# bobocode/lmono

Measured on AMD Instinct MI355X. Metric: KITTI HDL-64 scans/sec (scanRegistration + laserOdometry), higher is better.
Workload: dtype f32 features / f64 solve

## Files before the change

### lmono_amd/csrc/corr_flat.hip

```cpp
#include "batch.hpp"

namespace lmono {

#ifndef LMONO_CF_T
#define LMONO_CF_T 128
#endif
constexpr int kCfT = LMONO_CF_T;
constexpr int kCfBlocks = kMaxQueries / kCfT;
static_assert(kMaxQueries % kCfT == 0, "feature capacity must be a multiple of the workgroup size");
static_assert(kCfBlocks == kThinBlocks, "k_lm_solve skips the records of the workgroups a thinned lead-in pair does not run");
#ifndef LMONO_CF_PER
#define LMONO_CF_PER 6
#endif
#ifndef LMONO_CF_WAVES
#define LMONO_CF_WAVES 1
#endif
constexpr int kCfPer = LMONO_CF_PER;
constexpr int kCfPool = kCfT * kCfPer;
#ifndef LMONO_R0_PLANE
#define LMONO_R0_PLANE 0.25f
#define LMONO_R0_EDGE 0.7f
#endif
constexpr float kCfR0Edge = LMONO_R0_EDGE, kCfR0Plane = LMONO_R0_PLANE;
constexpr int kCfC = 4;
// ... 329 lines not shown
            elev_window(rr, elo, ehi);
            cf_window_extend(el, elo, ehi, v1, v2);
            const int pieces = cf_arc_pieces(a);
            const int nreq = max(v2 - v1 + 1, 0) * pieces;
            int slot = nreq > 0 ? atomicAdd(&L.n_pool[par], nreq) : 0;
            if (slot + nreq <= kCfPool) {
                posted = true;
                const int n0 = min(a.nb, kAzBins - a.a0);
                const unsigned int w0 = cf_request_line(0, a.a0, n0, tid), w1 = cf_request_line(0, 0, a.nb - n0, tid);
                for (int v = v1; v <= v2; v++) {
                    const float4 ev = el[v];
                    const bool meet = !(ev.y < elo || ev.x > ehi);
                    L.req[slot++] = meet ? (w0 | (unsigned int)v) : 0u;
                    if (pieces == 2) L.req[slot++] = meet ? (w1 | (unsigned int)v) : 0u;
                }
            } else {
                for (int t = slot; t < kCfPool; t++) L.req[t] = 0u;
            }
        }
        __syncthreads();
        CF_STAMP(cf_acc[0])
        const int n_chunks = cf_sweep<false>(L, par, n_edge_owner, tg, pts_c, pts_s, cf_t, cf_acc);
        par ^= 1;
        __syncthreads();
        CF_STAMP(cf_acc[2])
#ifdef LMONO_TILE_PROF
        if (tid == 0) { cf_acc[6] += 1; cf_acc[8] += (unsigned long long)n_chunks; }
#else
        (void)n_chunks;
#endif
        if (alive && posted) {
            const unsigned long long best = L.best[tid];
            if (best != ~0ull) {
                const float bd = __uint_as_float((unsigned int)(best >> 32));
                if (bd <= (rr * 0.9999f) * (rr * 0.9999f) || rr >= 5.0f) alive = false;
                else r = sqrtf(bd) * 1.0005f + 1e-3f;
            } else {
                if (rr >= 5.0f) alive = false;
                else r = rr * 2.5f;
            }
        }
        CF_STAMP(cf_acc[3])
        if (!__syncthreads_or(alive ? 1 : 0)) break;
    }
    if (alive) { alive = false; deferred = true; }

    const unsigned long long nn = L.best[tid];
    const unsigned long long thr = pack_fu(25.0f, 0u);
    bool walking = qi < nq && n_last > 0 && !deferred && nn != ~0ull && (double)__uint_as_float((unsigned int)(nn >> 32)) < 25.0;
    const int closest = (int)((unsigned int)(nn & 0xffffffffull) >> 7);
    const int ra = (int)(nn & 127ull);
    if (walking) {
        L.closest[tid] = (closest << 7) | ra;
        L.wlo[tid] = ra - 3 >= 0 ? L.lle[cl][ra - 3] + 1 : 0;
        L.whi[tid] = ra + 3 <= 65 ? L.fge[cl][ra + 3] : n_last;
    }
    const float rad[4] = { walk_radius(0, rho), walk_radius(1, rho), walk_radius(2, rho), walk_radius(3, rho) };
    int wpass = 0;
    unsigned long long same = thr, other = thr;
    float r_seed = -1.0f;
    if (walking && prev.w != 0 && prev.x == closest) {
        const int i_o = edge ? prev.y : prev.z;
        const float4 po = cloud[i_o];
        float d = dist2f(po.x, po.y, po.z, qx, qy, qz);
        if (!edge) { const float4 ps = cloud[prev.y]; d = fmaxf(d, dist2f(ps.x, ps.y, ps.z, qx, qy, qz)); }
        if (d < 24.0f) r_seed = sqrtf(d) * 1.002f + 1e-3f;
    }
    for (int round = 0; round < kCfWalkRounds; round++) {
#ifdef LMONO_TILE_PROF
        my_rounds += walking ? 1 : 0;
#endif
        bool posted = false;
        if (walking) {
            while (wpass > 0 && wpass < 4 && rad[wpass] <= rad[wpass - 1]) wpass++;
            if (wpass >= 4) walking = false;
        }
        const bool seeded = r_seed > 0.0f;
        const float r_now = seeded ? r_seed : rad[wpass < 4 ? wpass : 3];
        if (walking) {
            CfArc a;
            cf_arc(r_now, rho, th, a);
            const int wv1 = max(ra - 2, 0), wv2 = min(ra + 2, 65);
            const int nreq = (wv2 - wv1 + 1 - (edge ? 1 : 0)) * cf_arc_pieces(a);
            int slot = atomicAdd(&L.n_pool[par], nreq);
            if (slot + nreq <= kCfPool) {
                posted = true;
                L.same[tid] = thr; L.other[tid] = thr;
                for (int v = wv1; v <= wv2; v++) if (!(edge && v == ra)) cf_post_line(L.req, slot, a, v, tid);
            } else
                for (int t = slot; t < kCfPool; t++) L.req[t] = 0u;
        }
        __syncthreads();
        CF_STAMP(cf_acc[0])
        const int n_chunks = cf_sweep<true>(L, par, n_edge_owner, tg, pts_c, pts_s, cf_t, cf_acc);
        par ^= 1;
        __syncthreads();
        CF_STAMP(cf_acc[2])
#ifdef LMONO_TILE_PROF
        if (tid == 0) { cf_acc[7] += 1; cf_acc[9] += (unsigned long long)n_chunks; }
#else
        (void)n_chunks;
#endif
        if (walking && posted) {
            same = L.same[tid]; other = L.other[tid];
            if (!seeded && r_now >= 5.0f) walking = false;
            else {
                const unsigned long long lim = pack_fu(r_now * r_now * 0.998f, 0u);
                if (other < lim && (edge || same < lim)) walking = false;
                else if (seeded) r_seed = -1.0f;
                else {
                    wpass++;
                    while (wpass < 4 && rad[wpass] <= rad[wpass - 1]) wpass++;
                    if (other < thr && (edge || same < thr)) {
                        const float d = edge ? __uint_as_float((unsigned int)(other >> 32)) : fmaxf(__uint_as_float((unsigned int)(other >> 32)), __uint_as_float((unsigned int)(same >> 32)));
                        const float rt = sqrtf(d) * 1.002f + 1e-3f;
                        if (wpass < 4 && rt < rad[wpass] && d < 24.0f) r_seed = rt;
                    }
                }
            }
        }
        CF_STAMP(cf_acc[3])
        if (!__syncthreads_or(walking ? 1 : 0)) break;
    }
#ifdef LMONO_TILE_PROF
    {
        const int mr = __syncthreads_or(0) * 0 + my_rounds;
        __shared__ int s_maxr, s_sumr;
        if (tid == 0) { s_maxr = 0; s_sumr = 0; }
        __syncthreads();
        atomicMax(&s_maxr, mr); atomicAdd(&s_sumr, mr);
        __syncthreads();
        if (tid == 0) { cf_acc[17] = (unsigned long long)s_maxr; cf_acc[18] = (unsigned long long)s_sumr; }
    }
    if (tid == 0 && stats) { atomicAdd(&stats[1], 1ull); for (int i = 0; i < 20; i++) atomicAdd(&stats[2 + i], cf_acc[i]); }
#endif
    if (qi >= nq) return;
    if (deferred || walking) { cf_defer(wl, c, qi); return; }
    int4 rres = make_int4(-1, -1, -1, 0);
    int closest_out = -1;
    if (n_last > 0 && nn != ~0ull && (double)__uint_as_float((unsigned int)(nn >> 32)) < 25.0) {
        closest_out = closest;
        const int i_other = other < thr ? seq_to_index((unsigned int)(other & 0xffffffffull), closest) : -1;
        if (edge) { if (i_other >= 0) rres = make_int4(closest, i_other, -1, 1); }
        else {
            const int i_same = same < thr ? seq_to_index((unsigned int)(same & 0xffffffffull), closest) : -1;
            if (i_same >= 0 && i_other >= 0) rres = make_int4(closest, i_same, i_other, 2);
        }
    }
    ((int4 *)o.corr + (size_t)c * kMaxQueries)[qi] = rres;
    if (outer == 0 && seed_c) seed_c[qi] = closest_out;
    float4 A = make_float4(0.f, 0.f, 0.f, 0.f), B = A, C = A;
    if (rres.w != 0) { A = cloud[rres.x]; B = cloud[rres.y]; if (rres.z >= 0) C = cloud[rres.z]; }
    fp.w = __int_as_float(rres.w);
    float4 *rec = o.crec + ((size_t)c * kMaxQueries + qi) * 4;
    rec[0] = fp; rec[1] = A; rec[2] = B; rec[3] = C;
}

}
```

### lmono_amd/csrc/odometry.hip

```cpp
#include "batch.hpp"

namespace lmono {

constexpr float kCell = 1.0f;
constexpr float kInvCell = 1.0f;
constexpr int kMaxShell = 6;
constexpr int kCoordOff = 1 << 20;
constexpr int kRunMaxCount = 32767;
__device__ __forceinline__ int pack_run(int start, int count) { return start | (count << 17); }

__device__ __forceinline__ unsigned long long cell_key(int cx, int cy, int cz)
{
    return ((unsigned long long)(unsigned int)(cx + kCoordOff) << 42) |
           ((unsigned long long)(unsigned int)(cy + kCoordOff) << 21) |
           (unsigned long long)(unsigned int)(cz + kCoordOff);
}
__device__ __forceinline__ unsigned int hash_key(unsigned long long k)
{
    const unsigned int cz = (unsigned int)(k & 0x1fffffull), cy = (unsigned int)((k >> 21) & 0x1fffffull), cx = (unsigned int)(k >> 42);
    unsigned int h = (cx * 73856093u) ^ (cy * 19349663u) ^ (cz * 83492791u);
    h ^= h >> 15;
    return h;
}

struct GridRef {
    const GridCell *cell;
    const float4 *pts;
    int mask;
};

constexpr int kGridPage = 16384;
constexpr int kGridPar = 2;
constexpr int kGridLds = kGridPage * 8;
constexpr unsigned int kEmptyKey32 = 0xffffffffu;

__device__ __forceinline__ unsigned int grid_next(unsigned int sl, unsigned int pmask) { return (sl & ~pmask) | ((sl + 1) & pmask); }

__device__ __forceinline__ bool cell_key32(int cx, int cy, int cz, unsigned int &k)
{
    const unsigned int ux = (unsigned int)(cx + 1024), uy = (unsigned int)(cy + 1024), uz = (unsigned int)(cz + 512);
    k = ux | (uy << 11) | (uz << 22);
    return ux < 2048u && uy < 2048u && uz < 1023u;
}
__device__ __forceinline__ unsigned int hash_cell(int cx, int cy, int cz)
{
    unsigned int h = ((unsigned int)(cx + kCoordOff) * 73856093u) ^ ((unsigned int)(cy + kCoordOff) * 19349663u) ^ ((unsigned int)(cz + kCoordOff) * 83492791u);
    h ^= h >> 15;
    return h;
}
__device__ __forceinline__ unsigned long long key32_to_64(unsigned int k)
{
    return cell_key((int)(k & 2047u) - 1024, (int)((k >> 11) & 2047u) - 1024, (int)(k >> 22) - 512);
}

#ifdef LMONO_DIAG_SEARCH
__global__ __launch_bounds__(1024) void k_grid_build(BatchView b)
{
    const int s = b.scan0 + blockIdx.x;
    const bool surf = blockIdx.y > 0;
    const int tid = threadIdx.x, lane = tid & 63, wave = tid >> 6;
    const int n = b.feat_n[s * 4 + (surf ? 3 : 1)];
    const int Tcap = surf ? kSurfTable : kCornerTable;
    int T = next_pow2(n + 1);
    if (T < 1024) T = 1024;
    GridCell *cell = surf ? b.sg_cell + (size_t)s * kSurfTable : b.cg_cell + (size_t)s * kCornerTable;
    const int p0 = surf ? (int)blockIdx.y - 1 : 0, pstep = surf ? kGridPar : 1;
    if (T > Tcap) {
        if (p0 == 0) {
            for (int i = tid; i < 1024; i += 1024) { GridCell e; e.key = kEmptyKey; e.start = 0; e.cnt = 0; cell[i] = e; }
            if (tid == 0) { b.grid_mask[s * 2 + (surf ? 1 : 0)] = 1023; atomicOr(&b.status[s], kStatusGridOverflow); }
        }
        return;
    }
    const int P = T < kGridPage ? T : kGridPage, n_pages = T / P, pshift = __ffs(P) - 1;
    if (p0 >= n_pages) return;
    if (tid == 0 && p0 == 0) b.grid_mask[s * 2 + (surf ? 1 : 0)] = T - 1;
    const float4 *src = surf ? b.less_flat + b.off[s] : b.less_sharp + (size_t)s * kMaxLessSharp;
    float4 *dst = surf ? b.sg_pts + b.off[s] : b.cg_pts + (size_t)s * kMaxLessSharp;
    extern __shared__ __align__(16) unsigned int g_lds[];
    unsigned int *keys = g_lds;
    int *cnt = (int *)(g_lds + kGridPage);
    __shared__ int s_wsum[16], s_before, s_fail, s_occ;
    const unsigned int pm = (unsigned int)(P - 1);

    for (int p = p0; p < n_pages; p += pstep) {
        for (int i = tid; i < P; i += 1024) { keys[i] = kEmptyKey32; cnt[i] = 0; }
        if (tid == 0) { s_before = 0; s_fail = 0; s_occ = 0; }
        __syncthreads();
#pragma unroll
        for (int pass = 0; pass < 2; pass++) {
            int before = 0;
            bool fail = false;
            float4 nxt[4];
#pragma unroll
            for (int q = 0; q < 4; q++) { const int i = wave * 256 + 64 * q + lane; nxt[q] = i < n ? src[i] : make_float4(0.f, 0.f, 0.f, 0.f); }
            for (int t0 = wave * 256; t0 < n; t0 += 16 * 256) {
                unsigned int k32[4], sl[4];
                float4 pt[4];
                bool mine[4], head[4];
                int hl[4], len[4], base[4];
#pragma unroll
                for (int q = 0; q < 4; q++) {
                    pt[q] = nxt[q];
                    const int i = t0 + 16 * 256 + 64 * q + lane;
                    nxt[q] = i < n ? src[i] : make_float4(0.f, 0.f, 0.f, 0.f);
                }
#pragma unroll
                for (int q = 0; q < 4; q++) {
                    const int i = t0 + 64 * q + lane;
                    const int cx = (int)floorf(pt[q].x * kInvCell), cy = (int)floorf(pt[q].y * kInvCell), cz = (int)floorf(pt[q].z * kInvCell);
                    const bool ok = cell_key32(cx, cy, cz, k32[q]);
                    const unsigned int h = hash_cell(cx, cy, cz) & (unsigned int)(T - 1);
                    const int pg = (int)(h >> pshift);
                    sl[q] = h & pm;
                    mine[q] = i < n && pg == p;
                    if (i < n && pg < p) before++;
                    if (mine[q] && !ok) { fail = true; mine[q] = false; }
                }
#pragma unroll
                for (int q = 0; q < 4; q++) {
                    const unsigned int prev = (unsigned int)__shfl_up((int)k32[q], 1);
                    const unsigned long long mm = __ballot(mine[q]);
                    head[q] = mine[q] && (lane == 0 || !((mm >> (lane - 1)) & 1ull) || k32[q] != prev);
                    const unsigned long long hm = __ballot(head[q]);
                    hl[q] = 63 - __clzll((long long)(hm & ((2ull << lane) - 1ull)));
                    const unsigned long long stop = hm | ~mm;
                    const unsigned long long rest = lane < 63 ? stop >> (lane + 1) : 0ull;
                    len[q] = rest ? __ffsll((long long)rest) : 64 - lane;
                }
                unsigned int o4[4];
#pragma unroll
                for (int q = 0; q < 4; q++)
                    o4[q] = head[q] ? (pass == 0 ? atomicCAS(&keys[sl[q]], kEmptyKey32, k32[q]) : keys[sl[q]]) : k32[q];
#pragma unroll
                for (int q = 0; q < 4; q++) {
                    if (head[q]) {
                        unsigned int o = o4[q];
                        int tries = 0;
                        while (!(o == k32[q] || (pass == 0 && o == kEmptyKey32))) {
                            if (++tries >= P || (pass == 1 && o == kEmptyKey32)) { fail = true; head[q] = false; break; }
                            sl[q] = (sl[q] + 1) & pm;
                            o = pass == 0 ? atomicCAS(&keys[sl[q]], kEmptyKey32, k32[q]) : keys[sl[q]];
                        }
                    }
                }
#pragma unroll
                for (int q = 0; q < 4; q++) base[q] = head[q] ? atomicAdd(&cnt[sl[q]], len[q]) : -1;
                if (pass == 1) {
#pragma unroll
                    for (int q = 0; q < 4; q++) {
                        const int i = t0 + 64 * q + lane;
                        const int h = max(hl[q], 0);
                        const int b_run = __shfl(base[q], h);
// ... 371 lines not shown

template <bool kEdge>
__device__ __forceinline__ int4 correspond_g32(const BatchView &b, int k, int qi, const double *x, int gl, int gbase, int seed, int &closest_out)
{
    closest_out = -1;
    const int n_sharp = b.feat_n[k * 4 + 0];
    constexpr bool edge = kEdge;
    const float4 p = edge ? b.sharp[(size_t)k * kMaxSharp + qi] : b.flat[(size_t)k * kMaxFlat + (qi - n_sharp)];
    double rx, ry, rz;
    quat_rotate(x, (double)p.x, (double)p.y, (double)p.z, rx, ry, rz);
    const float qx = (float)(rx + x[4]), qy = (float)(ry + x[5]), qz = (float)(rz + x[6]);
    const int l = k - 1;
    const int cl = edge ? 0 : 1;
    const GridCell *cell = edge ? b.cg_cell + (size_t)l * kCornerTable : b.sg_cell + (size_t)l * kSurfTable;
    const float4 *gpts = edge ? b.cg_pts + (size_t)l * kMaxLessSharp : b.sg_pts + b.off[l];
    const float4 *lb_pts = edge ? b.lbc_pts + (size_t)l * kMaxLessSharp : b.lbs_pts + b.off[l];
    const int n_last = b.feat_n[l * 4 + (edge ? 1 : 3)];
    const unsigned int mask = (unsigned int)b.grid_mask[l * 2 + cl], pmask = min(mask, (unsigned int)(kGridPage - 1));
    int4 out = make_int4(-1, -1, -1, 0);
    if (n_last == 0) return out;

    const float fx = qx * kInvCell, fy = qy * kInvCell, fz = qz * kInvCell;
    const int cqx = (int)floorf(fx), cqy = (int)floorf(fy), cqz = (int)floorf(fz);
    int run = 0;
    bool near = false;
    NnBest nb = kNnNone;
    bool seeded = false;
    float sd = 0.f;
    if (seed >= 0 && seed < n_last) {
        const float4 pp = (edge ? b.less_sharp + (size_t)l * kMaxLessSharp : b.less_flat + b.off[l])[seed];
        const float d = dist2f(pp.x, pp.y, pp.z, qx, qy, qz);
        const int ln = (int)pp.w;
        if (d <= (kCell * 0.9999f) * (kCell * 0.9999f)) {
            seeded = true; sd = d;
            nb = ((unsigned long long)__float_as_uint(d) << 32) | (unsigned int)((seed << 7) | (ln < 0 ? 0 : (ln > 65 ? 65 : ln)));
        }
    }
    if (gl < 27 && b.has_grid) {
        const int dx = gl % 3 - 1, dy = (gl / 3) % 3 - 1, dz = gl / 9 - 1;
        const int sx = (fx - (float)cqx) >= 0.5f ? 1 : -1, sy = (fy - (float)cqy) >= 0.5f ? 1 : -1, sz = (fz - (float)cqz) >= 0.5f ? 1 : -1;
        near = (dx == 0 || dx == sx) && (dy == 0 || dy == sy) && (dz == 0 || dz == sz);
        bool wanted = true;
        if (seeded) {
            const float lx = (float)(cqx + dx) * kCell, ly = (float)(cqy + dy) * kCell, lz = (float)(cqz + dz) * kCell;
            const float ex = fmaxf(fmaxf(lx - qx, qx - (lx + kCell)), 0.f), ey = fmaxf(fmaxf(ly - qy, qy - (ly + kCell)), 0.f), ez = fmaxf(fmaxf(lz - qz, qz - (lz + kCell)), 0.f);
            const float eb = fmaxf(sqrtf(ex * ex + ey * ey + ez * ez) - 1e-3f, 0.f);
            wanted = !(eb * eb > sd);
        }
        if (wanted) {
            const unsigned long long kk = cell_key(cqx + dx, cqy + dy, cqz + dz);
            unsigned int sl = hash_key(kk) & mask;
            while (true) {
                const GridCell e = cell[sl];
                if (e.key == kk) { run = pack_run(e.start, e.cnt); break; }
                if (e.key == kEmptyKey) break;
                sl = grid_next(sl, pmask);
            }
        }
    }
    unsigned long long best;
    if (seeded) {
        nn_sweep(gpts, run, gl, gbase, qx, qy, qz, nb);
        best = group_min_u64(nb, gbase);
    } else {
    nn_sweep(gpts, near ? run : 0, gl, gbase, qx, qy, qz, nb);
    best = group_min_u64(nb, gbase);
    {
        const float bound_h = 0.5f * kCell * 0.9999f;
        if (!(best != ~0ull && __uint_as_float((unsigned int)(best >> 32)) <= bound_h * bound_h)) {
            int run_far = near ? 0 : run;
            if (best != ~0ull && gl < 27) {
                const float lx = (float)(cqx + gl % 3 - 1) * kCell, ly = (float)(cqy + (gl / 3) % 3 - 1) * kCell, lz = (float)(cqz + gl / 9 - 1) * kCell;
                const float ex = fmaxf(fmaxf(lx - qx, qx - (lx + kCell)), 0.f), ey = fmaxf(fmaxf(ly - qy, qy - (ly + kCell)), 0.f), ez = fmaxf(fmaxf(lz - qz, qz - (lz + kCell)), 0.f);
                const float eb = fmaxf(sqrtf(ex * ex + ey * ey + ez * ez) - 1e-3f, 0.f);
                if (eb * eb > __uint_as_float((unsigned int)(best >> 32))) run_far = 0;
            }
            nn_sweep(gpts, run_far, gl, gbase, qx, qy, qz, nb);
            best = group_min_u64(nb, gbase);
        }
    }
    }
    {
        const float bound = kCell * 0.9999f;
        const bool settled = b.has_grid && best != ~0ull && __uint_as_float((unsigned int)(best >> 32)) <= bound * bound;
        if (!settled) {
            const int *table = b.lb_start + (size_t)(l * 2 + cl) * (kLineKeys + 1);
            const float rho = sqrtf(qx * qx + qy * qy);
            const float th = atan2f(qy, qx) + 3.14159265f;
            const float bd = best != ~0ull ? __uint_as_float((unsigned int)(best >> 32)) : 25.0f;
            const float rr = bd < 25.0f ? sqrtf(bd) * 1.0005f + 1e-3f : 5.0f;
            int b_lo = 0, nbins = kAzBins;
            if (rho > rr * 1.002f) {
                const float alpha = asin_upper(rr / rho) + kArcSlackBins * (6.28318531f / kAzBins);
                const int lo = (int)floorf((th - alpha) * (kAzBins / 6.28318531f));
                const int hi = (int)floorf((th + alpha) * (kAzBins / 6.28318531f));
                if (hi - lo + 1 < kAzBins) { b_lo = ((lo % kAzBins) + kAzBins) % kAzBins; nbins = hi - lo + 1; }
            }
            lb_for_runs(table, b_lo, nbins, 0, 65, [&](int s0, int cn) { nn_sweep_arc(lb_pts, s0, cn, gl, qx, qy, qz, nb); });
            best = group_min_u64(nb, gbase);
        }
    }
    if (best == ~0ull || !((double)__uint_as_float((unsigned int)(best >> 32)) < 25.0)) return out;
    const int closest = (int)((unsigned int)(best & 0xffffffffull) >> 7);
    const int ra = (int)(best & 127ull);
    closest_out = closest;

    const int *fge = b.line_first_ge + (size_t)(l * 2 + cl) * 66;
    const int *lle = b.line_last_le + (size_t)(l * 2 + cl) * 66;
    const int *table = b.lb_start + (size_t)(l * 2 + cl) * (kLineKeys + 1);
    const float rho = sqrtf(qx * qx + qy * qy);
    const float th = atan2f(qy, qx) + 3.14159265f;
    const int w_lo = ra - 3 >= 0 ? lle[ra - 3] + 1 : 0;
    const int w_hi = ra + 3 <= 65 ? fge[ra + 3] : n_last;
    const unsigned long long thr = pack_fu(25.0f, 0u);
    unsigned long long same = thr, other = thr;
    float rprev = 0.f;
    for (int pass = (rho > 5.01f ? 0 : 3); pass < 4; pass++) {
        const float rw = walk_radius(pass, rho);
        if (rw <= rprev) continue;
        rprev = rw;
        int b_lo = 0, nbins = kAzBins;
        if (rho > 5.01f) {
            const float alpha = asin_upper(rw / rho) + kArcSlackBins * (6.28318531f / kAzBins);
            const int lo = (int)floorf((th - alpha) * (kAzBins / 6.28318531f));
            const int hi = (int)floorf((th + alpha) * (kAzBins / 6.28318531f));
            if (hi - lo + 1 < kAzBins) { b_lo = ((lo % kAzBins) + kAzBins) % kAzBins; nbins = hi - lo + 1; }
        }
        WalkBest bs = thr, bo = thr;
        lb_for_runs(table, b_lo, nbins, max(ra - 2, 0), min(ra + 2, 65), [&](int r0, int cnw) {
            for (int i = gl; i < cnw; i += 4 * kGroup) {
                float4 v4[4];
#pragma unroll
                for (int u = 0; u < 4; u++) v4[u] = lb_pts[r0 + min(i + u * kGroup, cnw - 1)];
#pragma unroll
                for (int u = 0; u < 4; u++) if (i + u * kGroup < cnw) walk_point(v4[u], ra, closest, w_lo, w_hi, edge, qx, qy, qz, bs, bo);
            }
        });
        same = group_min_u64(bs, gbase);
        other = group_min_u64(bo, gbase);
        if (rw >= 5.0f) break;
        const unsigned long long lim = pack_fu(rw * rw * 0.998f, 0u);
        if (other < lim && (edge || same < lim)) break;
    }
    const int i_other = other < thr ? seq_to_index((unsigned int)(other & 0xffffffffull), closest) : -1;
    if (edge) {
        if (i_other >= 0) out = make_int4(closest, i_other, -1, 1);
        return out;
    }
    const int i_same = same < thr ? seq_to_index((unsigned int)(same & 0xffffffffull), closest) : -1;
    if (i_same >= 0 && i_other >= 0) out = make_int4(closest, i_same, i_other, 2);
    return out;
}

__device__ __forceinline__ void correspond_group(const BatchView &b, const OdomView &o, int c, int k, int qi, int outer, int gl, int gbase)
{
    const int n_sharp = b.feat_n[k * 4 + 0];
    const int l = k - 1;
    int4 *corr = (int4 *)o.corr + (size_t)c * kMaxQueries;
    int *seed_c = o.seed ? o.seed + (size_t)c * kMaxQueries : nullptr;
    int closest;
    const int seed = (outer == 1 && seed_c) ? seed_c[qi] : -1;
    const double *x = o.state + c * 8;
    const int4 r = qi < n_sharp ? correspond_g32<true>(b, k, qi, x, gl, gbase, seed, closest) : correspond_g32<false>(b, k, qi, x, gl, gbase, seed, closest);
    if (gl == 0) { corr[qi] = r; if (outer == 0 && seed_c) seed_c[qi] = closest; }
    if (gl < 4) {
        const bool edge = qi < n_sharp;
        const float4 *cloud = edge ? b.less_sharp + (size_t)l * kMaxLessSharp : b.less_flat + b.off[l];
        float4 v = make_float4(0.f, 0.f, 0.f, 0.f);
        if (gl == 0) {
            v = edge ? b.sharp[(size_t)k * kMaxSharp + qi] : b.flat[(size_t)k * kMaxFlat + (qi - n_sharp)];
            v.w = __int_as_float(r.w);
        } else if (r.w != 0) {
            const int idx = gl == 1 ? r.x : (gl == 2 ? r.y : r.z);
            if (idx >= 0) v = cloud[idx];
        }
        o.crec[((size_t)c * kMaxQueries + qi) * 4 + gl] = v;
    }
}

__device__ __forceinline__ void correspond_wave(const BatchView &b, const OdomView &o, int c, int k, int qi, int lane)
{
    const int n_sharp = b.feat_n[k * 4 + 0];
    const int l = k - 1;
    int4 *corr = (int4 *)o.corr + (size_t)c * kMaxQueries;
    const double *x = o.state + c * 8;
    const int4 r = correspond_one(b, k, qi, x, lane);
    if (lane == 0) { corr[qi] = r; if (o.seed) o.seed[(size_t)c * kMaxQueries + qi] = -1; }
    if (lane < 4) {
        const bool edge = qi < n_sharp;
        const float4 *cloud = edge ? b.less_sharp + (size_t)l * kMaxLessSharp : b.less_flat + b.off[l];
        float4 v = make_float4(0.f, 0.f, 0.f, 0.f);
        if (lane == 0) { v = edge ? b.sharp[(size_t)k * kMaxSharp + qi] : b.flat[(size_t)k * kMaxFlat + (qi - n_sharp)]; v.w = __int_as_float(r.w); }
        else if (r.w != 0) { const int idx = lane == 1 ? r.x : (lane == 2 ? r.y : r.z); if (idx >= 0) v = cloud[idx]; }
        o.crec[((size_t)c * kMaxQueries + qi) * 4 + lane] = v;
    }
}

constexpr int kCorrBlocks = kMaxQueries / 8;

#ifdef LMONO_DIAG_SEARCH
__global__ __launch_bounds__(256, 8) void k_correspond(BatchView b, OdomView o, int step, int outer)
{
    const int xcd = blockIdx.x & 7, u = blockIdx.x >> 3;
    const int c = o.chain0 + (u / kCorrBlocks) * 8 + xcd;
    const int qblock = u % kCorrBlocks;
    if (c >= o.chain1) return;
    const int lane = threadIdx.x & 63;
    const int gl = threadIdx.x & (kGroup - 1), gbase = lane & ~(kGroup - 1);
    int own;
    const int k = chain_scan(o, c, step, own);
    if (k < 0) return;
    const int n_sharp = b.feat_n[k * 4 + 0];
    const int nq = n_sharp + b.feat_n[k * 4 + 2];
    const double *x = o.state + c * 8;
    int4 *corr = (int4 *)o.corr + (size_t)c * kMaxQueries;
    const int l = k - 1;
    if (b.status[l] & (kStatusIrregularLines | kStatusDenseCell)) {
        for (int t = 0; t < 2; t++) {
            const int qi = qblock * 8 + (threadIdx.x >> 6) * 2 + t;
            if (qi >= nq) break;
            correspond_wave(b, o, c, k, qi, lane);
        }
        return;
    }
    const int qi = qblock * 8 + (threadIdx.x >> 5);
    if (qi >= nq) return;
    correspond_group(b, o, c, k, qi, outer, gl, gbase);
}
#endif

__global__ __launch_bounds__(256, 4) void k_correspond_list(BatchView b, OdomView o, int step, int outer, const unsigned int *wl, unsigned long long *stats)
{
    const unsigned int n = wl[0];
    if (blockIdx.x == 0 && threadIdx.x == 0 && stats && n) atomicAdd(&stats[0], (unsigned long long)n);
    const int lane = threadIdx.x & 63;
    const int gl = threadIdx.x & (kGroup - 1), gbase = lane & ~(kGroup - 1);
    for (unsigned int it = blockIdx.x * 8 + (threadIdx.x >> 5); it < n; it += gridDim.x * 8) {
        const unsigned int e = wl[1 + it];
        const int c = (int)(e >> 12), qi = (int)(e & 4095u);
        int own;
        const int k = chain_scan(o, c, step, own);
        if (k < 0 || (b.status[k - 1] & (kStatusIrregularLines | kStatusDenseCell))) continue;
        correspond_group(b, o, c, k, qi, outer, gl, gbase);
    }
    for (unsigned int it = blockIdx.x * 4 + (threadIdx.x >> 6); it < n; it += gridDim.x * 4) {
        const unsigned int e = wl[1 + it];
        const int c = (int)(e >> 12), qi = (int)(e & 4095u);
        int own;
        const int k = chain_scan(o, c, step, own);
        if (k < 0 || !(b.status[k - 1] & (kStatusIrregularLines | kStatusDenseCell))) continue;
        correspond_wave(b, o, c, k, qi, lane);
    }
}

constexpr int kLmT = 256;
constexpr int kLmW = kLmT / 64;
__device__ __forceinline__ void stage_block(const float4 cp, const float4 A, const float4 B, const float4 Cc, double *P)
{
    const int kind = __float_as_int(cp.w);
    if (kind == 1) {
        const double ex = (double)A.x - (double)B.x, ey = (double)A.y - (double)B.y, ez = (double)A.z - (double)B.z;
        const double inv = 1.0 / sqrt(ex * ex + ey * ey + ez * ez);
        P[0] = (double)A.x; P[1] = (double)A.y; P[2] = (double)A.z;
        P[3] = ex * inv; P[4] = ey * inv; P[5] = ez * inv;
    } else {
        const double jx = (double)A.x, jy = (double)A.y, jz = (double)A.z;
        const double ux = jx - (double)B.x, uy = jy - (double)B.y, uz = jz - (double)B.z;
        const double wx = jx - (double)Cc.x, wy = jy - (double)Cc.y, wz = jz - (double)Cc.z;
        double nx = uy * wz - uz * wy, ny = uz * wx - ux * wz, nz = ux * wy - uy * wx;
        const double nn = sqrt(nx * nx + ny * ny + nz * nz);
        if (nn > 0.0) { nx /= nn; ny /= nn; nz /= nn; }
        P[0] = jx; P[1] = jy; P[2] = jz; P[3] = nx; P[4] = ny; P[5] = nz;
    }
}

__device__ __forceinline__ void lm_row(LmAcc &acc, double d0, double d1, double d2, double rvx, double rvy, double rvz, double res, double sr)
{
#pragma clang fp contract(fast)
    double J[6];
    const double s2 = 2.0 * sr;
    J[0] = (rvy * d2 - rvz * d1) * s2; J[1] = (rvz * d0 - rvx * d2) * s2; J[2] = (rvx * d1 - rvy * d0) * s2;
    J[3] = d0 * sr; J[4] = d1 * sr; J[5] = d2 * sr;
    accumulate_row(acc, J, res * sr);
}

template <bool kJac, bool kEdge>
__device__ __forceinline__ void eval_block(const float4 cp, const double2 P01, const double2 P23, const double2 P45, const double *Rm, const double *x, LmAcc &acc)
{
#pragma clang fp contract(fast)
    if (__float_as_int(cp.w) == 0) return;
    const double vx = (double)cp.x, vy = (double)cp.y, vz = (double)cp.z;
    const double rvx = Rm[0] * vx + Rm[1] * vy + Rm[2] * vz, rvy = Rm[3] * vx + Rm[4] * vy + Rm[5] * vz, rvz = Rm[6] * vx + Rm[7] * vy + Rm[8] * vz;
    const double dx = rvx + x[4] - P01.x, dy = rvy + x[5] - P01.y, dz = rvz + x[6] - P23.x;
    const double qx = P23.y, qy = P45.x, qz = P45.y;
    double r0, r1 = 0.0, r2 = 0.0, sq;
    if (kEdge) { r0 = dy * qz - dz * qy; r1 = dz * qx - dx * qz; r2 = dx * qy - dy * qx; sq = r0 * r0 + r1 * r1 + r2 * r2; }
    else { r0 = dx * qx + dy * qy + dz * qz; sq = r0 * r0; }
    double rho0, rho1;
    huber(sq, rho0, rho1);
    acc.cost += 0.5 * rho0;
    if (!kJac) return;
    const double sr = rho1 == 1.0 ? 1.0 : sqrt(rho1);
    if (kEdge) {
        lm_row(acc, 0.0, qz, -qy, rvx, rvy, rvz, r0, sr);
        lm_row(acc, -qz, 0.0, qx, rvx, rvy, rvz, r1, sr);
        lm_row(acc, qy, -qx, 0.0, rvx, rvy, rvz, r2, sr);
    } else
        lm_row(acc, qx, qy, qz, rvx, rvy, rvz, r0, sr);
}

struct LmBlk { float4 cp; double2 p01, p23, p45; };
template <int kPlanes>
struct LmRec {
    static_assert(kPlanes == 0 || kPlanes == 4, "the instantiations the library holds");
    float4 *lds;
    float4 *mem;
    template <int p> __device__ __forceinline__ float4 *plane() const { return p < kPlanes ? lds + p * kMaxQueries : mem + (p - kPlanes) * kMaxQueries; }
    __device__ __forceinline__ void put(int qi, const float4 cp, const double *P) const
    {
        plane<0>()[qi] = cp;
        ((double2 *)plane<1>())[qi] = make_double2(P[0], P[1]);
        ((double2 *)plane<2>())[qi] = make_double2(P[2], P[3]);
        ((double2 *)plane<3>())[qi] = make_double2(P[4], P[5]);
    }
    __device__ __forceinline__ void request(int qi, LmBlk &k) const
    {
        if (kPlanes < 1) k.cp = plane<0>()[qi];
        if (kPlanes < 2) k.p01 = ((const double2 *)plane<1>())[qi];
        if (kPlanes < 3) k.p23 = ((const double2 *)plane<2>())[qi];
        if (kPlanes < 4) k.p45 = ((const double2 *)plane<3>())[qi];
    }
    __device__ __forceinline__ void local(int qi, LmBlk &k) const
    {
        if (kPlanes >= 1) k.cp = plane<0>()[qi];
        if (kPlanes >= 2) k.p01 = ((const double2 *)plane<1>())[qi];
        if (kPlanes >= 3) k.p23 = ((const double2 *)plane<2>())[qi];
        if (kPlanes >= 4) k.p45 = ((const double2 *)plane<3>())[qi];
    }
};

template <bool kJac, int kPlanes>
__device__ __forceinline__ void evaluate_block(const LmRec<kPlanes> rec, int n_edge, int nq, const double *x, double (*s_red)[28], double *s_sum)
{
    const int tid = threadIdx.x, lane = tid & 63, wave = tid >> 6;
    LmAcc acc;
    acc.cost = 0.0;
    if (kJac) {
#pragma unroll
        for (int i = 0; i < 21; i++) acc.H[i] = 0.0;
#pragma unroll
        for (int i = 0; i < 6; i++) acc.g[i] = 0.0;
    }
    double Rm[9];
    {
#pragma clang fp contract(fast)
        const double ux = x[0], uy = x[1], uz = x[2], w = x[3];
        Rm[0] = 1.0 - 2.0 * (uy * uy + uz * uz); Rm[1] = 2.0 * (ux * uy - w * uz);       Rm[2] = 2.0 * (ux * uz + w * uy);
        Rm[3] = 2.0 * (ux * uy + w * uz);       Rm[4] = 1.0 - 2.0 * (ux * ux + uz * uz); Rm[5] = 2.0 * (uy * uz - w * ux);
        Rm[6] = 2.0 * (ux * uz - w * uy);       Rm[7] = 2.0 * (uy * uz + w * ux);       Rm[8] = 1.0 - 2.0 * (ux * ux + uy * uy);
    }
    int qi = tid;
    if (kPlanes == 4) {
        const float4 *srec = rec.lds;
        const double2 *sp = (const double2 *)srec;
        for (; qi < n_edge; qi += kLmT)
            eval_block<kJac, true>(srec[qi], sp[kMaxQueries + qi], sp[2 * kMaxQueries + qi], sp[3 * kMaxQueries + qi], Rm, x, acc);
        for (; qi < nq; qi += kLmT)
            eval_block<kJac, false>(srec[qi], sp[kMaxQueries + qi], sp[2 * kMaxQueries + qi], sp[3 * kMaxQueries + qi], Rm, x, acc);
    } else {
        LmBlk cur = {}, nxt;
        if (qi < nq) rec.request(qi, cur);
        for (; qi < n_edge; qi += kLmT) {
            nxt = cur;
            if (qi + kLmT < nq) rec.request(qi + kLmT, nxt);
            rec.local(qi, cur);
            eval_block<kJac, true>(cur.cp, cur.p01, cur.p23, cur.p45, Rm, x, acc);
            cur = nxt;
        }
        for (; qi < nq; qi += kLmT) {
            nxt = cur;
            if (qi + kLmT < nq) rec.request(qi + kLmT, nxt);
            rec.local(qi, cur);
            eval_block<kJac, false>(cur.cp, cur.p01, cur.p23, cur.p45, Rm, x, acc);
            cur = nxt;
        }
    }
    acc.cost = wave_sum_d(acc.cost);
    if (kJac) {
#pragma unroll
        for (int i = 0; i < 21; i++) acc.H[i] = wave_sum_d(acc.H[i]);
#pragma unroll
        for (int i = 0; i < 6; i++) acc.g[i] = wave_sum_d(acc.g[i]);
    }
    __syncthreads();
    if (lane == 0) {
        s_red[wave][27] = acc.cost;
        if (kJac) {
            for (int i = 0; i < 21; i++) s_red[wave][i] = acc.H[i];
            for (int i = 0; i < 6; i++) s_red[wave][21 + i] = acc.g[i];
        }
    }
    __syncthreads();
    if (tid < 28 && (kJac || tid == 27)) {
        double t = 0.0;
        for (int w = 0; w < kLmW; w++) t += s_red[w][tid];
        s_sum[tid] = t;
    }
    __syncthreads();
}

constexpr int lm_rec_lds(int planes) { return planes * kMaxQueries * 16; }
constexpr int kLmPlanesDefault = 0;
__host__ inline bool lm_planes_valid(int planes) { return planes == 4 || planes == 0; }
#ifndef LMONO_LM_VGPRS
#define LMONO_LM_VGPRS 240
#endif
#ifndef LMONO_CF_T
#define LMONO_CF_T 128
#endif
constexpr int kThinBlocks = kMaxQueries / LMONO_CF_T;

#ifndef LMONO_LM_MAX_ITER
#define LMONO_LM_MAX_ITER 4
#endif

template <int kPlanes>
__global__ __launch_bounds__(kLmT) __attribute__((amdgpu_num_vgpr(LMONO_LM_VGPRS / 2))) void k_lm_solve(BatchView b, OdomView o, int step, int outer, unsigned int *wl_reset)
{
    const int c = o.clist ? o.clist[o.chain0 + blockIdx.x] : o.chain0 + (int)blockIdx.x;
    if (wl_reset && blockIdx.x == 0 && threadIdx.x == 0) wl_reset[0] = 0u;
    int s;
    const int k = chain_scan(o, c, step, s);
    if (k < 0) return;
    __shared__ double s_red[kLmW][28], s_sum[28], s_cur[28];
    __shared__ int s_used[kLmW];
    const int tid = threadIdx.x, lane = tid & 63, wave = tid >> 6;
    const int n_edge = b.feat_n[k * 4 + 0], nq = n_edge + b.feat_n[k * 4 + 2];
    const float4 *crec = o.crec + (size_t)c * kMaxQueries * 4;
    extern __shared__ __align__(16) float4 s_rec[];
    const LmRec<kPlanes> rec = { s_rec, kPlanes < 4 ? o.lmrec + (size_t)c * (4 - kPlanes) * kMaxQueries : nullptr };
    int n_used = 0;
    {
        const bool thin = lead_in_thinned(o, k, s);
        for (int qi = tid; qi < nq; qi += kLmT) {
            float4 cp = crec[qi * 4];
            const float4 A = crec[qi * 4 + 1], B = crec[qi * 4 + 2], Cc = crec[qi * 4 + 3];
            if (thin && (qi % kThinBlocks) % kThinStride != 0) cp.w = 0.f;
            double P[6] = { 0.0, 0.0, 0.0, 0.0, 0.0, 0.0 };
            if (__float_as_int(cp.w) != 0) { stage_block(cp, A, B, Cc, P); n_used++; }
            rec.put(qi, cp, P);
        }
    }
    __syncthreads();
    double x[7];
    for (int i = 0; i < 7; i++) x[i] = o.state[c * 8 + i];

    evaluate_block<true>(rec, n_edge, nq, x, s_red, s_sum);
    n_used = wave_sum_i(n_used);
    if (lane == 0) s_used[wave] = n_used;
    __syncthreads();
    n_used = 0;
    for (int w = 0; w < kLmW; w++) n_used += s_used[w];
    TrustRegion<true> tr(LMONO_LM_MAX_ITER);
    auto take = [&]() {
        __syncthreads();
        if (tid < 28) s_cur[tid] = s_sum[tid];
        __syncthreads();
    };
    if (tid < 28) s_cur[tid] = s_sum[tid];
    __syncthreads();
    if (n_used > 0 && tr.begin(s_cur, x))
        for (;;) {
            double cand[7];
            if (tr.propose(s_cur, x, cand) == 2) break;
            if (tr.last()) evaluate_block<false>(rec, n_edge, nq, cand, s_red, s_sum);
            else evaluate_block<true>(rec, n_edge, nq, cand, s_red, s_sum);
            if (!tr.judge(s_sum, s_cur, x, cand, take)) break;
        }
    if (tid == 0) {
        for (int i = 0; i < 7; i++) o.state[c * 8 + i] = x[i];
        if (o.repair && outer == 1) {
            int e0, e1;
            chain_bounds(o.first, o.n_scans, o.n_chains, c, e0, e1);
            const double res = boundary_residual(x, o.incr + (size_t)k * 7);
            for (int i = 0; i < 7; i++) o.incr[(size_t)k * 7 + i] = x[i];
            o.rstat[c * 4 + 1] += 1;
            int agree = o.rstat[c * 4 + 2] >> 1;
            agree = res <= o.tol ? agree + 1 : 0;
            o.rstat[c * 4 + 2] = 1 | (agree << 1);
            if (agree >= kRepairAgree || k + 1 >= e1) { o.rstat[c * 4] = 1; atomicSub(&o.rcount[1], 1u); }
        } else if (o.incr && outer == 1 && k >= s)
            for (int i = 0; i < 7; i++) o.incr[(size_t)k * 7 + i] = x[i];
        if (o.ws && !o.repair && outer == 1 && k == s - 1)
            for (int i = 0; i < 7; i++) o.ws[c * 8 + i] = x[i];
        if (o.lm_info) { o.lm_info[c * 4 + outer] = tr.iter; o.lm_info[c * 4 + 2 + outer] = n_used; }
    }
}

__global__ __launch_bounds__(256) void k_boundary_check(OdomView o, double *resid, int first_round, int ext)
{
    __shared__ int s_n;
    if (threadIdx.x == 0) s_n = 0;
    __syncthreads();
    for (int base = 0; base < o.n_chains; base += 256) {
        const int c = base + threadIdx.x;
        bool flag = false;
        if (c < o.n_chains) {
            int s, e;
            chain_bounds(o.first, o.n_scans, o.n_chains, c, s, e);
            double res = 0.0;
            if ((c > 0 || ext) && s > 0) res = boundary_residual(o.ws + c * 8, o.incr + (size_t)(s - 1) * 7);
            if (resid) resid[c] = res;
            flag = res > o.tol;
            if (first_round) { o.rstat[c * 4 + 1] = 0; o.rstat[c * 4 + 3] = 0; }
            o.rstat[c * 4] = flag ? 0 : 1;
            o.rstat[c * 4 + 2] = flag ? 1 : 0;
            if (flag) {
                o.rstat[c * 4 + 3] += 1;
                for (int i = 0; i < 7; i++) { const double v = o.incr[(size_t)(s - 1) * 7 + i]; o.state[c * 8 + i] = v; o.ws[c * 8 + i] = v; }
            }
        }
        const unsigned long long m = __ballot(flag);
        __shared__ int s_w[4];
        if ((threadIdx.x & 63) == 0) s_w[threadIdx.x >> 6] = __popcll(m);
        __syncthreads();
        int pre = s_n;
        for (int w = 0; w < (int)(threadIdx.x >> 6); w++) pre += s_w[w];
        if (flag) o.rcount[2 + pre + __popcll(m & ((1ull << (threadIdx.x & 63)) - 1ull))] = (unsigned int)c;
        __syncthreads();
        if (threadIdx.x == 0) s_n += s_w[0] + s_w[1] + s_w[2] + s_w[3];
        __syncthreads();
    }
    if (threadIdx.x == 0) { o.rcount[0] = (unsigned int)s_n; o.rcount[1] = (unsigned int)s_n; }
}

__global__ void k_odom_init(OdomView o)
{
    const int i = blockIdx.x * blockDim.x + threadIdx.x;
    if (i < o.n_chains) {
        double *st = o.state + i * 8;
        st[0] = st[1] = st[2] = 0.0; st[3] = 1.0; st[4] = st[5] = st[6] = 0.0; st[7] = 0.0;
        if (o.ws) { double *w = o.ws + i * 8; w[0] = w[1] = w[2] = 0.0; w[3] = 1.0; w[4] = w[5] = w[6] = 0.0; w[7] = 0.0; }
    }
    if (i < o.n_scans) {
        double *r = o.incr + (size_t)i * 7;
        r[0] = r[1] = r[2] = 0.0; r[3] = 1.0; r[4] = r[5] = r[6] = 0.0;
    }
}

__device__ __forceinline__ double median3(double a, double b, double c) { return fmax(fmin(a, b), fmin(fmax(a, b), c)); }
__device__ __forceinline__ bool chain_seeded(const OdomView &o, int c)
{
    int s, e;
    chain_bounds(o.first, o.n_scans, o.n_chains, c, s, e);
    const int begin = max(s - o.lead, 0);
    return begin + 1 < s - 1;
}
__global__ void k_lead_seed_median(OdomView o)
{
    const int c = blockIdx.x * blockDim.x + threadIdx.x;
    if (c >= o.n_chains || !chain_seeded(o, c)) return;
    const int c0 = min(max(c - 1, 0), max(o.n_chains - 3, 0));
    double v[3][7];
    for (int j = 0; j < 3; j++) {
        const double *st = o.state + (size_t)min(c0 + j, o.n_chains - 1) * 8;
        const double sg = st[3] < 0.0 ? -1.0 : 1.0;
        for (int i = 0; i < 4; i++) v[j][i] = sg * st[i];
        for (int i = 4; i < 7; i++) v[j][i] = st[i];
    }
    double m[7], nn = 0.0;
    for (int i = 0; i < 7; i++) m[i] = median3(v[0][i], v[1][i], v[2][i]);
    for (int i = 0; i < 4; i++) nn += m[i] * m[i];
    nn = sqrt(nn);
    const bool ok = nn > 0.5 && nn == nn;
    for (int i = 0; i < 4; i++) o.ws[c * 8 + i] = ok ? m[i] / nn : o.state[c * 8 + i];
    for (int i = 4; i < 7; i++) o.ws[c * 8 + i] = ok && m[i] == m[i] ? m[i] : o.state[c * 8 + i];
}
__global__ void k_lead_seed_apply(OdomView o)
{
    const int c = blockIdx.x * blockDim.x + threadIdx.x;
    if (c >= o.n_chains || !chain_seeded(o, c)) return;
    for (int i = 0; i < 7; i++) o.state[c * 8 + i] = o.ws[c * 8 + i];
}

__device__ __forceinline__ void se3_compose(const double *a, const double *b, double *o)
{
    double rx, ry, rz;
    quat_rotate(a, b[4], b[5], b[6], rx, ry, rz);
    const double ax = a[0], ay = a[1], az = a[2], aw = a[3];
    const double bx = b[0], by = b[1], bz = b[2], bw = b[3];
    const double t0 = a[4] + rx, t1 = a[5] + ry, t2 = a[6] + rz;
    o[3] = aw * bw - ax * bx - ay * by - az * bz;
    o[0] = aw * bx + ax * bw + ay * bz - az * by;
    o[1] = aw * by + ay * bw + az * bx - ax * bz;
    o[2] = aw * bz + az * bw + ax * by - ay * bx;
    o[4] = t0; o[5] = t1; o[6] = t2;
}

__global__ __launch_bounds__(64) void k_pose_prefix(const double *incr, double *poses, int first, int n)
{
    const int lane = threadIdx.x;
    incr += (size_t)first * 7;
// ... 54 lines not shown
```

Measured before the change: 135,400.

## Stage line/plane parameters in correspondence kernels and scatter-reduce LM sums

Correspondence kernels now compute each edge or plane's anchor point and unit direction or normal in f64 and store them in the staged record, replacing the raw neighbour points. The LM kernel then reads these precomputed doubles instead of recomputing stage_block on every solve. The per-wave reduction of the 28 Hessian, gradient and cost sums is replaced by a scatter-reduce built on permlane swaps and DPP/swizzle exchanges, which leaves one result per lane pair instead of running 28 separate full wave reductions. In exchange the correspondence kernels do the f64 normalisation on a single lane rather than spreading the record writes across four lanes, and the code now depends on permlane16/32 swap builtins.

Result: faster. 138,500, median of 6 (+2.3%).

```diff
diff --git a/lmono_amd/csrc/corr_flat.hip b/lmono_amd/csrc/corr_flat.hip
--- a/lmono_amd/csrc/corr_flat.hip
+++ b/lmono_amd/csrc/corr_flat.hip
@@ -505,8 +505,7 @@
     float4 A = make_float4(0.f, 0.f, 0.f, 0.f), B = A, C = A;
     if (rres.w != 0) { A = cloud[rres.x]; B = cloud[rres.y]; if (rres.z >= 0) C = cloud[rres.z]; }
     fp.w = __int_as_float(rres.w);
-    float4 *rec = o.crec + ((size_t)c * kMaxQueries + qi) * 4;
-    rec[0] = fp; rec[1] = A; rec[2] = B; rec[3] = C;
-}
-
-}
+    store_staged_record(o.crec + ((size_t)c * kMaxQueries + qi) * 4, fp, A, B, C);
+}
+
+}
diff --git a/lmono_amd/csrc/odometry.hip b/lmono_amd/csrc/odometry.hip
--- a/lmono_amd/csrc/odometry.hip
+++ b/lmono_amd/csrc/odometry.hip
@@ -1,4 +1,5 @@
 #include "batch.hpp"
+#include "wave_sum28.hpp"
 
 namespace lmono {
 
@@ -676,6 +677,35 @@
     return out;
 }
 
+__device__ __forceinline__ void stage_block(const float4 cp, const float4 A, const float4 B, const float4 Cc, double *P)
+{
+    const int kind = __float_as_int(cp.w);
+    if (kind == 1) {
+        const double ex = (double)A.x - (double)B.x, ey = (double)A.y - (double)B.y, ez = (double)A.z - (double)B.z;
+        const double inv = 1.0 / sqrt(ex * ex + ey * ey + ez * ez);
+        P[0] = (double)A.x; P[1] = (double)A.y; P[2] = (double)A.z;
+        P[3] = ex * inv; P[4] = ey * inv; P[5] = ez * inv;
+    } else {
+        const double jx = (double)A.x, jy = (double)A.y, jz = (double)A.z;
+        const double ux = jx - (double)B.x, uy = jy - (double)B.y, uz = jz - (double)B.z;
+        const double wx = jx - (double)Cc.x, wy = jy - (double)Cc.y, wz = jz - (double)Cc.z;
+        double nx = uy * wz - uz * wy, ny = uz * wx - ux * wz, nz = ux * wy - uy * wx;
+        const double nn = sqrt(nx * nx + ny * ny + nz * nz);
+        if (nn > 0.0) { nx /= nn; ny /= nn; nz /= nn; }
+        P[0] = jx; P[1] = jy; P[2] = jz; P[3] = nx; P[4] = ny; P[5] = nz;
+    }
+}
+
+__device__ __forceinline__ void store_staged_record(float4 *rec, const float4 cp, const float4 A, const float4 B, const float4 Cc)
+{
+    double P[6] = { 0.0, 0.0, 0.0, 0.0, 0.0, 0.0 };
+    if (__float_as_int(cp.w) != 0) stage_block(cp, A, B, Cc, P);
+    rec[0] = cp;
+    ((double2 *)rec)[1] = make_double2(P[0], P[1]);
+    ((double2 *)rec)[2] = make_double2(P[2], P[3]);
+    ((double2 *)rec)[3] = make_double2(P[4], P[5]);
+}
+
 __device__ __forceinline__ void correspond_group(const BatchView &b, const OdomView &o, int c, int k, int qi, int outer, int gl, int gbase)
 {
     const int n_sharp = b.feat_n[k * 4 + 0];
@@ -687,18 +717,14 @@
     const double *x = o.state + c * 8;
     const int4 r = qi < n_sharp ? correspond_g32<true>(b, k, qi, x, gl, gbase, seed, closest) : correspond_g32<false>(b, k, qi, x, gl, gbase, seed, closest);
     if (gl == 0) { corr[qi] = r; if (outer == 0 && seed_c) seed_c[qi] = closest; }
-    if (gl < 4) {
+    if (gl == 0) {
         const bool edge = qi < n_sharp;
         const float4 *cloud = edge ? b.less_sharp + (size_t)l * kMaxLessSharp : b.less_flat + b.off[l];
-        float4 v = make_float4(0.f, 0.f, 0.f, 0.f);
-        if (gl == 0) {
-            v = edge ? b.sharp[(size_t)k * kMaxSharp + qi] : b.flat[(size_t)k * kMaxFlat + (qi - n_sharp)];
-            v.w = __int_as_float(r.w);
-        } else if (r.w != 0) {
-            const int idx = gl == 1 ? r.x : (gl == 2 ? r.y : r.z);
-            if (idx >= 0) v = cloud[idx];
-        }
-        o.crec[((size_t)c * kMaxQueries + qi) * 4 + gl] = v;
+        float4 cp = edge ? b.sharp[(size_t)k * kMaxSharp + qi] : b.flat[(size_t)k * kMaxFlat + (qi - n_sharp)];
+        cp.w = __int_as_float(r.w);
+        float4 A = make_float4(0.f, 0.f, 0.f, 0.f), B = A, Cc = A;
+        if (r.w != 0) { if (r.x >= 0) A = cloud[r.x]; if (r.y >= 0) B = cloud[r.y]; if (r.z >= 0) Cc = cloud[r.z]; }
+        store_staged_record(o.crec + ((size_t)c * kMaxQueries + qi) * 4, cp, A, B, Cc);
     }
 }
 
@@ -710,13 +736,14 @@
     const double *x = o.state + c * 8;
     const int4 r = correspond_one(b, k, qi, x, lane);
     if (lane == 0) { corr[qi] = r; if (o.seed) o.seed[(size_t)c * kMaxQueries + qi] = -1; }
-    if (lane < 4) {
+    if (lane == 0) {
         const bool edge = qi < n_sharp;
         const float4 *cloud = edge ? b.less_sharp + (size_t)l * kMaxLessSharp : b.less_flat + b.off[l];
-        float4 v = make_float4(0.f, 0.f, 0.f, 0.f);
-        if (lane == 0) { v = edge ? b.sharp[(size_t)k * kMaxSharp + qi] : b.flat[(size_t)k * kMaxFlat + (qi - n_sharp)]; v.w = __int_as_float(r.w); }
-        else if (r.w != 0) { const int idx = lane == 1 ? r.x : (lane == 2 ? r.y : r.z); if (idx >= 0) v = cloud[idx]; }
-        o.crec[((size_t)c * kMaxQueries + qi) * 4 + lane] = v;
+        float4 cp = edge ? b.sharp[(size_t)k * kMaxSharp + qi] : b.flat[(size_t)k * kMaxFlat + (qi - n_sharp)];
+        cp.w = __int_as_float(r.w);
+        float4 A = make_float4(0.f, 0.f, 0.f, 0.f), B = A, Cc = A;
+        if (r.w != 0) { if (r.x >= 0) A = cloud[r.x]; if (r.y >= 0) B = cloud[r.y]; if (r.z >= 0) Cc = cloud[r.z]; }
+        store_staged_record(o.crec + ((size_t)c * kMaxQueries + qi) * 4, cp, A, B, Cc);
     }
 }
 
@@ -779,25 +806,6 @@
 
 constexpr int kLmT = 256;
 constexpr int kLmW = kLmT / 64;
-__device__ __forceinline__ void stage_block(const float4 cp, const float4 A, const float4 B, const float4 Cc, double *P)
-{
-    const int kind = __float_as_int(cp.w);
-    if (kind == 1) {
-        const double ex = (double)A.x - (double)B.x, ey = (double)A.y - (double)B.y, ez = (double)A.z - (double)B.z;
-        const double inv = 1.0 / sqrt(ex * ex + ey * ey + ez * ez);
-        P[0] = (double)A.x; P[1] = (double)A.y; P[2] = (double)A.z;
-        P[3] = ex * inv; P[4] = ey * inv; P[5] = ez * inv;
-    } else {
-        const double jx = (double)A.x, jy = (double)A.y, jz = (double)A.z;
-        const double ux = jx - (double)B.x, uy = jy - (double)B.y, uz = jz - (double)B.z;
-        const double wx = jx - (double)Cc.x, wy = jy - (double)Cc.y, wz = jz - (double)Cc.z;
-        double nx = uy * wz - uz * wy, ny = uz * wx - ux * wz, nz = ux * wy - uy * wx;
-        const double nn = sqrt(nx * nx + ny * ny + nz * nz);
-        if (nn > 0.0) { nx /= nn; ny /= nn; nz /= nn; }
-        P[0] = jx; P[1] = jy; P[2] = jz; P[3] = nx; P[4] = ny; P[5] = nz;
-    }
-}
-
 __device__ __forceinline__ void lm_row(LmAcc &acc, double d0, double d1, double d2, double rvx, double rvy, double rvz, double res, double sr)
 {
 #pragma clang fp contract(fast)
@@ -909,20 +917,22 @@
             cur = nxt;
         }
     }
-    acc.cost = wave_sum_d(acc.cost);
     if (kJac) {
-#pragma unroll
-        for (int i = 0; i < 21; i++) acc.H[i] = wave_sum_d(acc.H[i]);
-#pragma unroll
-        for (int i = 0; i < 6; i++) acc.g[i] = wave_sum_d(acc.g[i]);
-    }
-    __syncthreads();
-    if (lane == 0) {
-        s_red[wave][27] = acc.cost;
-        if (kJac) {
-            for (int i = 0; i < 21; i++) s_red[wave][i] = acc.H[i];
-            for (int i = 0; i < 6; i++) s_red[wave][21 + i] = acc.g[i];
-        }
+        double v[32];
+#pragma unroll
+        for (int i = 0; i < 21; i++) v[i] = acc.H[i];
+#pragma unroll
+        for (int i = 0; i < 6; i++) v[21 + i] = acc.g[i];
+        v[27] = acc.cost;
+#pragma unroll
+        for (int i = 28; i < 32; i++) v[i] = 0.0;
+        wave_sum28_scatter(Ws28Wave{ lane }, v);
+        __syncthreads();
+        if (!(lane & 1) && lane < 56) s_red[wave][lane >> 1] = v[0];
+    } else {
+        acc.cost = wave_sum_d(acc.cost);
+        __syncthreads();
+        if (lane == 0) s_red[wave][27] = acc.cost;
     }
     __syncthreads();
     if (tid < 28 && (kJac || tid == 27)) {
@@ -968,10 +978,10 @@
         const bool thin = lead_in_thinned(o, k, s);
         for (int qi = tid; qi < nq; qi += kLmT) {
             float4 cp = crec[qi * 4];
-            const float4 A = crec[qi * 4 + 1], B = crec[qi * 4 + 2], Cc = crec[qi * 4 + 3];
+            const double2 p01 = ((const double2 *)crec)[qi * 4 + 1], p23 = ((const double2 *)crec)[qi * 4 + 2], p45 = ((const double2 *)crec)[qi * 4 + 3];
             if (thin && (qi % kThinBlocks) % kThinStride != 0) cp.w = 0.f;
-            double P[6] = { 0.0, 0.0, 0.0, 0.0, 0.0, 0.0 };
-            if (__float_as_int(cp.w) != 0) { stage_block(cp, A, B, Cc, P); n_used++; }
+            if (__float_as_int(cp.w) != 0) n_used++;
+            const double P[6] = { p01.x, p01.y, p23.x, p23.y, p45.x, p45.y };
             rec.put(qi, cp, P);
         }
     }
diff --git a/lmono_amd/csrc/wave_sum28.hpp b/lmono_amd/csrc/wave_sum28.hpp
--- /dev/null
+++ b/lmono_amd/csrc/wave_sum28.hpp
@@ -0,0 +1,83 @@
+#pragma once
+
+#if defined(__HIPCC__)
+#define LMONO_WS28_HD __host__ __device__ __forceinline__
+#else
+#define LMONO_WS28_HD inline
+#endif
+
+namespace lmono {
+
+template <int kMask, int kHalf, class L, class T>
+LMONO_WS28_HD void ws28_stage_swap(const L &lanes, T *v)
+{
+#pragma unroll
+    for (int j = 0; j < kHalf; j++) {
+        lanes.template swap<kMask>(v[j], v[j + kHalf]);
+        v[j] = v[j] + v[j + kHalf];
+    }
+}
+
+template <int kMask, int kHalf, class L, class T>
+LMONO_WS28_HD void ws28_stage_xchg(const L &lanes, T *v)
+{
+#pragma unroll
+    for (int j = 0; j < kHalf; j++) {
+        const T keep = lanes.template pick<kMask>(v[j], v[j + kHalf]);
+        const T send = lanes.template pick<kMask>(v[j + kHalf], v[j]);
+        v[j] = keep + lanes.template xchg<kMask>(send);
+    }
+}
+
+template <class L, class T>
+LMONO_WS28_HD void wave_sum28_scatter(const L &lanes, T *v)
+{
+    ws28_stage_swap<32, 16>(lanes, v);
+    ws28_stage_swap<16, 8>(lanes, v);
+    ws28_stage_xchg<8, 4>(lanes, v);
+    ws28_stage_xchg<4, 2>(lanes, v);
+    ws28_stage_xchg<2, 1>(lanes, v);
+    v[0] = v[0] + lanes.template xchg<1>(v[0]);
+}
+
+#if defined(__HIPCC__)
+struct Ws28Wave {
+    int lane;
+    template <int kMask> __device__ __forceinline__ double pick(double a, double b) const { return (lane & kMask) ? b : a; }
+    template <int kMask> __device__ __forceinline__ static unsigned int xchg32(unsigned int u)
+    {
+        static_assert(kMask == 8 || kMask == 4 || kMask == 2 || kMask == 1, "the masks the scatter exchanges by moves");
+        if (kMask == 8) return (unsigned int)__builtin_amdgcn_update_dpp(0, (int)u, 0x128, 0xf, 0xf, false);
+        if (kMask == 4) return (unsigned int)__builtin_amdgcn_ds_swizzle((int)u, 0x101f);
+        if (kMask == 2) return (unsigned int)__builtin_amdgcn_update_dpp(0, (int)u, 0x4e, 0xf, 0xf, false);
+        return (unsigned int)__builtin_amdgcn_update_dpp(0, (int)u, 0xb1, 0xf, 0xf, false);
+    }
+    template <int kMask> __device__ __forceinline__ double xchg(double a) const
+    {
+        const unsigned long long u = (unsigned long long)__double_as_longlong(a);
+        const unsigned int lo = xchg32<kMask>((unsigned int)u), hi = xchg32<kMask>((unsigned int)(u >> 32));
+        return __longlong_as_double((long long)(((unsigned long long)hi << 32) | lo));
+    }
+    template <int kMask> __device__ __forceinline__ void swap(double &a, double &b) const
+    {
+        static_assert(kMask == 32 || kMask == 16, "the masks that have a swap instruction");
+        const unsigned long long ua = (unsigned long long)__double_as_longlong(a), ub = (unsigned long long)__double_as_longlong(b);
+        unsigned int alo = (unsigned int)ua, ahi = (unsigned int)(ua >> 32), blo = (unsigned int)ub, bhi = (unsigned int)(ub >> 32);
+        if (kMask == 32) {
+            const auto l = __builtin_amdgcn_permlane32_swap(alo, blo, false, false);
+            const auto h = __builtin_amdgcn_permlane32_swap(ahi, bhi, false, false);
+            alo = l[0]; blo = l[1]; ahi = h[0]; bhi = h[1];
+        } else {
+            const auto l = __builtin_amdgcn_permlane16_swap(alo, blo, false, false);
+            const auto h = __builtin_amdgcn_permlane16_swap(ahi, bhi, false, false);
+            alo = l[0]; blo = l[1]; ahi = h[0]; bhi = h[1];
+        }
+        a = __longlong_as_double((long long)(((unsigned long long)ahi << 32) | alo));
+        b = __longlong_as_double((long long)(((unsigned long long)bhi << 32) | blo));
+    }
+};
+#endif
+
+}
+
+#undef LMONO_WS28_HD
```
